# THUDM/GCC

Hardware: AMD Instinct MI355X
Metric: sampled-subgraphs/sec (higher is better)
Workload: dtype f32

## Files before the change

gcc_amd/_cabi.py:

```python
from __future__ import annotations

import ctypes
import os

_HERE = os.path.dirname(os.path.abspath(__file__))
LIB_PATH = os.path.join(_HERE, "csrc", "libgcc_amd.so")
HEADER_PATH = os.path.join(os.path.dirname(_HERE), "include", "gcc_amd.h")

c_i32p = ctypes.POINTER(ctypes.c_int32)
c_f32p = ctypes.POINTER(ctypes.c_float)
c_f64p = ctypes.POINTER(ctypes.c_double)

STATUS_SCRATCH_OVERFLOW = 1
STATUS_NODE_OVERFLOW = 2
STATUS_EDGE_OVERFLOW = 4


class GccGraph(ctypes.Structure):
    _fields_ = [
        ("row_ptr", ctypes.c_void_p),
        ("col_idx", ctypes.c_void_p),
        ("seed_cdf", ctypes.c_void_p),
        ("ltab", ctypes.c_void_p),
        ("num_nodes", ctypes.c_int64),
# ... 227 lines not shown
                                          ctypes.c_void_p, ctypes.c_void_p, ctypes.c_void_p, ctypes.c_void_p]),
    "gcc_posemb": (ctypes.c_int32, [ctypes.POINTER(GccBatchOut), ctypes.c_int32, ctypes.c_int32, ctypes.c_void_p,
                                    ctypes.c_void_p, ctypes.c_void_p, ctypes.c_uint64, ctypes.c_void_p, ctypes.c_int64, ctypes.c_void_p,
                                    ctypes.c_void_p, ctypes.c_void_p]),
    "gcc_gin_forward": (ctypes.c_int32, [ctypes.POINTER(GccGinPass), ctypes.c_int32, ctypes.c_void_p,
                                         ctypes.c_void_p]),
    "gcc_gin_forward_fetch": (ctypes.c_int32, [ctypes.POINTER(GccGinPass), ctypes.c_int32, ctypes.c_void_p, ctypes.c_void_p,
                                               ctypes.c_int32, ctypes.c_void_p, ctypes.c_void_p, ctypes.c_void_p]),
    "gcc_gin_backward_workspace_bytes": (ctypes.c_int64, [ctypes.c_int64, ctypes.c_int32, ctypes.c_int32]),
    "gcc_gin_backward": (ctypes.c_int32, [ctypes.POINTER(GccGinPass), ctypes.c_void_p, ctypes.POINTER(GccGinGrads),
                                          ctypes.c_int32, ctypes.c_void_p, ctypes.c_int64, ctypes.c_int64,
                                          ctypes.c_void_p, ctypes.c_void_p]),
    "gcc_gin_backward_sumsq": (ctypes.c_int32, [ctypes.POINTER(GccGinPass), ctypes.c_void_p, ctypes.POINTER(GccGinGrads),
                                                ctypes.c_void_p, ctypes.c_int64, ctypes.c_int64, ctypes.c_void_p, ctypes.c_int32,
                                                c_i32p, ctypes.c_void_p, ctypes.c_void_p]),
    "gcc_ginx_workspace_bytes": (ctypes.c_int64, [ctypes.c_int64, ctypes.c_int32, ctypes.c_int32, ctypes.c_int32, ctypes.c_int32, ctypes.c_int32]),
    "gcc_ginx_forward": (ctypes.c_int32, [ctypes.POINTER(GccGinxPass), ctypes.c_void_p]),
    "gcc_ginx_backward": (ctypes.c_int32, [ctypes.POINTER(GccGinxPass), ctypes.c_void_p, ctypes.POINTER(GccGinGrads), ctypes.c_void_p]),
    "gcc_ncex_forward": (ctypes.c_int32, [ctypes.c_void_p, ctypes.c_void_p, ctypes.c_void_p, ctypes.c_int32, ctypes.c_int32, ctypes.c_int32,
                                          ctypes.c_float, ctypes.c_int32] + [ctypes.c_void_p] * 8),
    "gcc_queue_enqueue_x": (ctypes.c_int32, [ctypes.c_void_p, ctypes.c_int32, ctypes.c_int32, ctypes.c_void_p, ctypes.c_int32, ctypes.c_int32,
                                             ctypes.c_void_p]),
    "gcc_ginw_forward": (ctypes.c_int32, [ctypes.POINTER(GccGinwArgs), ctypes.c_void_p, ctypes.c_void_p, ctypes.c_void_p]),
    "gcc_ginw_pack_weights": (ctypes.c_int32, [ctypes.c_void_p, ctypes.c_void_p, ctypes.c_int32, ctypes.c_void_p]),
    "gcc_nce_workspace_bytes": (ctypes.c_int64, [ctypes.c_int32, ctypes.c_int32]),
    "gcc_nce_forward": (ctypes.c_int32, [ctypes.POINTER(GccNceArgs), ctypes.c_void_p, ctypes.c_int64,
                                         ctypes.c_void_p, ctypes.c_void_p]),
    "gcc_nce_backward": (ctypes.c_int32, [ctypes.POINTER(GccNceArgs), ctypes.c_void_p, ctypes.c_int32,
                                          ctypes.c_void_p, ctypes.c_void_p, ctypes.c_int64, ctypes.c_void_p,
                                          ctypes.c_void_p]),
# ... 100 lines not shown
```

gcc_amd/csrc/encoder_bwd.hip:

```cpp
#include "encoder_common.h"

namespace {

constexpr int kWgChunks = 64;

struct BnCol { float mean, rstd, gamma, beta; };
__device__ __forceinline__ BnCol bn_col(const BnDev &bn, int c, double s1, double s2, double n, float eps)
{
    const double mean = s1 / n;
    double var = s2 / n - mean * mean;
    if (var < 0.0) var = 0.0;
    BnCol r;
    r.mean = (float)mean;
    r.rstd = (float)(1.0 / sqrt(var + (double)eps));
    r.gamma = bn.weight[c];
    r.beta = bn.bias[c];
    return r;
}

enum { RS = 0, RM = 1, PS = 2, PH = 3, K1 = 4, K2 = 5, K3 = 6, kCoefRows = 7 };

__device__ __forceinline__ void fill_coefs(float *C , const BnDev &bn, const double *bst, double n,
                                           float eps, double *scratch)
{
// ... 172 lines not shown
            g[cb] = gg;
            if (valid) st4(a.G + ((int64_t)i * a.B + b) * H + ch, gg);
        }
        f32x4 acc[4];
        mfma_rows16(g, wf, acc);
        if (valid) {
#pragma unroll
            for (int cb = 0; cb < 4; ++cb) {
                F4 o = {acc[cb][0], acc[cb][1], acc[cb][2], acc[cb][3]};
                st4(a.dpooled + ((int64_t)i * a.B + b) * H + 16 * cb + 4 * q, o);
            }
        }
    }
}

struct BwdCArgs {
    const int32_t *node_off, *row_ptr, *col_idx, *graph_id;
    const float *D;
    const float *dpooled;
    const float *z2;
    BnDev bnb, bnc;
    float *U;
    double *bst_c;
    int32_t B;
    float eps;
    int32_t cap;
};

#ifndef BWD_C_PER_CU
#define BWD_C_PER_CU 3
#endif
#ifndef BWD_GATHER_J
#define BWD_GATHER_J 8
#endif
__global__ __launch_bounds__(kThreads, BWD_C_PER_CU) void gin_bwd_c_kernel(BwdCArgs a)
{
    TRAIN_STEP_WAVE_PRIORITY();
    __shared__ float T[kTile * kLdt];
    __shared__ __attribute__((aligned(16))) float part[16 * 2 * H];
    __shared__ float Cb[kCoefRows * H], Cc[kCoefRows * H];
    __shared__ int prow[32];
    __shared__ int rpl[kTile + 1];
    const int tid = (int)threadIdx.x, t = tid & 15, gi = tid >> 4;
    int N;
    const float *Dp = a.D ? a.D : a.z2;
    auto ident = [&](int u) -> F4 { return ld4(Dp + (int64_t)u * H + 4 * t); };
    const int tf = first_tile();
    int gid4[kTile / 16], rp_own = 0;
    F4 own[kTile / 16], z4[kTile / 16];
    auto request = [&](int tile0) {
#pragma unroll
        for (int i = 0; i < kTile / 16; ++i) gid4[i] = a.graph_id[cap_row(tile0 + gi + 16 * i, a.cap)];
        rp_own = a.row_ptr[min(tile0 + min(tid, kTile), a.cap)];
#pragma unroll
        for (int i = 0; i < kTile / 16; ++i) own[i] = ident(cap_row(tile0 + gi + 16 * i, a.cap));
#pragma unroll
        for (int i = 0; i < kTile / 16; ++i) z4[i] = ld4(a.z2 + (int64_t)cap_row(tile0 + gi + 16 * i, a.cap) * H + 4 * t);
    };
    if (a.bnb.totals && a.bnc.totals) {
        const CoefReq rb = coef_request(a.bnb), rc = coef_request(a.bnc);
        const RepReq none = {};
        request(tf * kTile);
        N = a.node_off[a.B];
        SCHED_FENCE();
        if (no_tiles(N)) return;
        fill_coefs_from<false>(Cb, rb, none, (double)N, a.eps, (double *)part);
        fill_coefs_from<false>(Cc, rc, none, (double)N, a.eps, (double *)part);
        __syncthreads();
    } else {
        request(tf * kTile);
        N = ((const volatile int32_t *)a.node_off)[a.B];
        fill_coefs(Cb, a.bnb, nullptr, (double)N, a.eps, (double *)part);
        fill_coefs(Cc, a.bnc, nullptr, (double)N, a.eps, (double *)part);
    }
    F4 s1 = zero4(), s2 = zero4();
    bool any = false;
    for (TileWalk tw(N); tw.ti < tw.tend; tw.ti += tw.step) {
        const int tile0 = tw.ti * kTile;
        any = true;
        const int nrows = min(kTile, N - tile0);
        if (tw.ti != tf) request(tile0);
        F4 g4[kTile / 16];
        auto pooled_path = [&] {
#pragma unroll
            for (int i = 0; i < kTile / 16; ++i) g4[i] = ld4(a.dpooled + (int64_t)min(max(gid4[i], 0), a.B - 1) * H + 4 * t);
        };
        if (a.D) {
            if (tid <= nrows) rpl[tid] = rp_own;
#pragma unroll
            for (int i = 0; i < kTile / 16; ++i) st4(&T[(gi + 16 * i) * kLdt + 4 * t], gi + 16 * i < nrows ? own[i] : zero4());
            __syncthreads();
            gather_tile<BWD_GATHER_J>(T, part, prow, nrows, a.col_idx, ident, [](F4 x) { return x; }, 1.0f, rpl, pooled_path);
        } else {
            pooled_path();
        }
        {
            const F4 pbs = ld4(&Cb[PS * H + 4 * t]), pbh = ld4(&Cb[PH * H + 4 * t]);
            const F4 rcs = ld4(&Cc[RS * H + 4 * t]), rcm = ld4(&Cc[RM * H + 4 * t]);
            const F4 pcs = ld4(&Cc[PS * H + 4 * t]), pch = ld4(&Cc[PH * H + 4 * t]);
#pragma unroll
            for (int i = 0; i < kTile / 16; ++i) {
                const int r = gi + 16 * i, v = tile0 + r;
                if (r < nrows) {
                    F4 g = g4[i];
                    if (a.D) g = add4(g, ld4(&T[r * kLdt + 4 * t]));
                    const F4 y2 = relu4(fma4(z4[i], pbs, pbh));
                    const F4 yh = fma4(y2, rcs, rcm);
                    const F4 u = mask4(g, fma4(y2, pcs, pch));
                    st4(a.U + (int64_t)v * H + 4 * t, u);
                    s1 = add4(s1, u);
                    s2 = fma4(u, yh, s2);
                }
            }
        }
        __syncthreads();
    }
    if (!any) return;
    reduce_groups(part, s1, s2, a.bst_c, a.bst_c + H);
}

struct BwdBArgs {
    const int32_t *node_off;
    const float *U, *z2;
    BnDev bnb, bnc;
// ... 178 lines not shown
            else if (kMask) atomicAdd(&a.bst_out[rep + tid], v);
        }
        __syncthreads();
    }
}

constexpr int kEmbBlocks = 448;
constexpr int kEmbMaxElems = 10240;

struct EmbArgs {
    const int32_t *node_off, *row_ptr, *col_idx, *graph_id;
    const float *D, *dpooled0;
    float *demb_parts;
    int32_t B, pos_dim, emb_dim, max_degree;
    int32_t cap;
};

__global__ __launch_bounds__(kThreads) void gin_bwd_emb_kernel(EmbArgs a)
{
    TRAIN_STEP_WAVE_PRIORITY();
    __shared__ float T[kTile * kLdt];
    __shared__ float part[32 * H];
    __shared__ float E[kEmbMaxElems];
    __shared__ int dclrow[kTile], gidl[kTile];
    __shared__ int prow[32];
    __shared__ int rpl[kTile + 1];
    const int tid = (int)threadIdx.x, t = tid & 15, gi = tid >> 4;
    const bool my_cols = 4 * t + 3 >= a.pos_dim && 4 * t < a.pos_dim + a.emb_dim;
    auto ident = [&](int u) -> F4 { return my_cols ? ld4(a.D + (int64_t)u * H + 4 * t) : zero4(); };
    const int tf = first_tile();
    int rp_own, gid_own;
    F4 own[kTile / 16];
    auto request = [&](int tile0) {
        rp_own = a.row_ptr[min(tile0 + min(tid, kTile), a.cap)];
        gid_own = a.graph_id[cap_row(tile0 + (tid & (kTile - 1)), a.cap)];
#pragma unroll
        for (int i = 0; i < kTile / 16; ++i) own[i] = ident(cap_row(tile0 + gi + 16 * i, a.cap));
    };
    request(tf * kTile);
    const int N = a.node_off[a.B];
    SCHED_FENCE();
    const int elems = (a.max_degree + 1) * a.emb_dim;
    for (int i = tid; i < elems; i += kThreads) E[i] = 0.f;
    for (TileWalk tw(N); tw.ti < tw.tend; tw.ti += tw.step) {
        const int tile0 = tw.ti * kTile;
        const int nrows = min(kTile, N - tile0);
        {
            if (tw.ti != tf) request(tile0);
            if (tid <= nrows) rpl[tid] = rp_own;
            if (tid >= 128 && tid - 128 < nrows) gidl[tid - 128] = gid_own;
#pragma unroll
            for (int i = 0; i < kTile / 16; ++i) st4(&T[(gi + 16 * i) * kLdt + 4 * t], gi + 16 * i < nrows ? own[i] : zero4());
        }
        __syncthreads();
        constexpr int kIt = 4;
        const int total = nrows * a.emb_dim;
        int rr[kIt], cc[kIt];
        float dv[kIt];
        auto pooled_request = [&](int base) {
// ... 9 lines not shown
        if (tid < nrows) {
            const int deg = rpl[tid + 1] - rpl[tid];
            dclrow[tid] = deg < a.max_degree ? deg : a.max_degree;
        }
        for (int base = 0; base < total; base += kIt * kThreads) {
            if (base) pooled_request(base);
#pragma unroll
            for (int i = 0; i < kIt; ++i)
                if (base + tid + i * kThreads < total) T[rr[i] * kLdt + a.pos_dim + cc[i]] += dv[i];
        }
        __syncthreads();
        if (tid < a.emb_dim)
            for (int r = 0; r < nrows; ++r) E[dclrow[r] * a.emb_dim + tid] += T[r * kLdt + a.pos_dim + tid];
        __syncthreads();
    }
    for (int i = tid; i < elems; i += kThreads) a.demb_parts[(int64_t)blockIdx.x * elems + i] = E[i];
}

struct WgradJob {
    const float *dZ, *X;
    const double *Xd;
    BnDev bn;
    int32_t rows_fixed;
};
constexpr int kMaxWgJobs = 3 * GCC_GIN_MAX_LAYERS + 1;
struct WgradArgs {
    const int32_t *node_off;
    WgradJob job[kMaxWgJobs];
    float *slabs;
    float *bias_slabs;
    int32_t B;
    float eps;
    int32_t cap;
};

__global__ __launch_bounds__(kThreads, 3) void gin_wgrad_kernel(WgradArgs a)
{
    TRAIN_STEP_WAVE_PRIORITY();
    __shared__ float S[H * H];
    __shared__ float Cx[2 * H];
    const int jid = (int)blockIdx.y;
    const WgradJob &jb = a.job[jid];
    const int tid = (int)threadIdx.x, lane = lane_id(), wv = tid >> 6, j = lane & 15, q = lane >> 4;
    __shared__ float Sb[4 * H];
    const bool act = jb.bn.weight != nullptr;
    const bool fast = act && jb.bn.totals != nullptr;
    const int cc = tid & (H - 1);
    const double *tp = fast ? jb.bn.totals : (const double *)a.slabs;
    const float *wp = fast ? jb.bn.weight : a.slabs, *bp = fast ? jb.bn.bias : a.slabs;
    const CoefReq cr = {tp[cc], tp[H + cc], wp[cc], bp[cc]};
    const int rcap = jb.rows_fixed > 0 ? jb.rows_fixed : a.cap;
    f32x4 acc[4][4];
    float bsum[4] = {0.f, 0.f, 0.f, 0.f};
#pragma unroll
    for (int ob = 0; ob < 4; ++ob)
#pragma unroll
        for (int kb = 0; kb < 4; ++kb) { f32x4 z = {0.f, 0.f, 0.f, 0.f}; acc[ob][kb] = z; }
    float av[4][4], xv[4][4];
    const bool xdouble = jb.Xd != nullptr;
    auto fetch = [&](int tile0, float (&A)[4][4], float (&X)[4][4]) {
        int64_t off[4];
#pragma unroll
        for (int s = 0; s < 4; ++s) {
            const int row = tile0 + 16 * wv + 4 * s + q;
            off[s] = (int64_t)cap_row(row, rcap) * H + j;
#pragma unroll
            for (int k = 0; k < 4; ++k) A[s][k] = jb.dZ[off[s] + 16 * k];
        }
        if (xdouble) {
#pragma unroll
            for (int h = 0; h < 4; h += 2) {
                double xd[2][4];
#pragma unroll
                for (int s = 0; s < 2; ++s)
#pragma unroll
                    for (int k = 0; k < 4; ++k) xd[s][k] = jb.Xd[off[h + s] + 16 * k];
#pragma unroll
                for (int s = 0; s < 2; ++s)
#pragma unroll
                    for (int k = 0; k < 4; ++k) X[h + s][k] = (float)xd[s][k];
            }
        } else {
#pragma unroll
            for (int s = 0; s < 4; ++s)
#pragma unroll
                for (int k = 0; k < 4; ++k) X[s][k] = jb.X[off[s] + 16 * k];
        }
    };
    auto mask_tile = [&](int tile0, int N, float (&A)[4][4], float (&X)[4][4]) {
#pragma unroll
        for (int s = 0; s < 4; ++s) {
            const bool in = tile0 + 16 * wv + 4 * s + q < N;
#pragma unroll
            for (int k = 0; k < 4; ++k) { A[s][k] = in ? A[s][k] : 0.f; X[s][k] = in ? X[s][k] : 0.f; }
        }
    };
    const int tf = first_tile();
    fetch(tf * kTile, av, xv);
    const int Nn = a.node_off[a.B];
    SCHED_FENCE();
    const int N = jb.rows_fixed > 0 ? jb.rows_fixed : Nn;
    TileWalk tw(N);
    if (tid < H) {
        float sc = 1.f, sh = 0.f;
        if (fast) {
            const double mean = cr.s1 / (double)Nn;
            double var = cr.s2 / (double)Nn - mean * mean;
            if (var < 0.0) var = 0.0;
            const double rstd = 1.0 / sqrt(var + (double)a.eps);
            sc = (float)((double)cr.gamma * rstd);
            sh = (float)((double)cr.beta - mean * (double)cr.gamma * rstd);
        } else if (act) {
            bn_scale_shift(jb.bn, tid, (double)Nn, a.eps, 1, sc, sh);
        }
        Cx[tid] = sc;
        Cx[H + tid] = sh;
    }
    __syncthreads();
    float xs[4], xh[4];
#pragma unroll
    for (int kb = 0; kb < 4; ++kb) { xs[kb] = Cx[16 * kb + j]; xh[kb] = Cx[H + 16 * kb + j]; }
    for (; tw.ti < tw.tend; tw.ti += tw.step) {
        const int tile0 = tw.ti * kTile;
        float an[4][4], xn[4][4];
        const bool more = tw.ti + tw.step < tw.tend;
        if (more) fetch((tw.ti + tw.step) * kTile, an, xn);
        mask_tile(tile0, N, av, xv);
#pragma unroll
        for (int s = 0; s < 4; ++s) {
            const int row = tile0 + 16 * wv + 4 * s + q;
            float bv[4];
#pragma unroll
            for (int k = 0; k < 4; ++k) {
                bsum[k] += av[s][k];
                bv[k] = act ? (row < N ? fmaxf(fmaf(xv[s][k], xs[k], xh[k]), 0.f) : 0.f) : xv[s][k];
            }
#pragma unroll
            for (int ob = 0; ob < 4; ++ob)
#pragma unroll
                for (int kb = 0; kb < 4; ++kb) acc[ob][kb] = mfma_16x16x4_f32(av[s][ob], bv[kb], acc[ob][kb]);
        }
        if (more) {
#pragma unroll
            for (int s = 0; s < 4; ++s)
#pragma unroll
                for (int k = 0; k < 4; ++k) { av[s][k] = an[s][k]; xv[s][k] = xn[s][k]; }
        }
    }
    for (int w = 0; w < 4; ++w) {
        if (wv == w) {
#pragma unroll
            for (int ob = 0; ob < 4; ++ob)
#pragma unroll
                for (int kb = 0; kb < 4; ++kb)
#pragma unroll
                    for (int r = 0; r < 4; ++r) {
                        const int o = 16 * ob + 4 * q + r, k = 16 * kb + j;
                        S[o * H + k] = (w == 0 ? 0.f : S[o * H + k]) + acc[ob][kb][r];
                    }
        }
        __syncthreads();
    }
    float *slab = a.slabs + ((int64_t)jid * kWgChunks + blockIdx.x) * H * H;
    for (int i = tid; i < H * H; i += kThreads) slab[i] = S[i];
#pragma unroll
    for (int k = 0; k < 4; ++k) {
        bsum[k] += wave_shfl_xor(bsum[k], 16);
        bsum[k] += wave_shfl_xor(bsum[k], 32);
        if (q == 0) Sb[wv * H + 16 * k + j] = bsum[k];
    }
    __syncthreads();
    if (tid < H)
        a.bias_slabs[((int64_t)jid * kWgChunks + blockIdx.x) * H + tid] =
            (Sb[tid] + Sb[H + tid]) + (Sb[2 * H + tid] + Sb[3 * H + tid]);
}

struct FinalArgs {
    const float *slabs, *bias_slabs;
    const double *bst;
    const float *demb_parts;
    gcc_gin_grads g;
    int32_t B, L, kdim0, emb_rows, emb_dim, accumulate, hid;
    double *sumsq_parts;
};

__device__ __forceinline__ float put(float *dst, float v, int acc)
{
    if (!dst) return 0.f;
    const float w = acc ? *dst + v : v;
// ... 114 lines not shown
    w.total = o;
    return w;
}

}

extern "C" int64_t gcc_gin_backward_workspace_bytes(int64_t node_cap, int32_t batch_size, int32_t num_gin_layers)
{
    if (node_cap <= 0 || batch_size <= 0 || num_gin_layers < 1 || num_gin_layers > GCC_GIN_MAX_LAYERS) {
        snprintf(g_err, kErrLen, "gcc_gin_backward_workspace_bytes: bad argument");
        return -1;
    }
    return bwd_layout(nullptr, node_cap, batch_size, num_gin_layers, kEmbMaxElems).total;
}

static int32_t gin_backward_launches(const gcc_gin_pass *pass, const float *dfeat, const gcc_gin_grads *grads,
                                     int32_t accumulate, void *workspace, int64_t workspace_bytes,
                                     int64_t node_cap, double *sumsq_parts, int32_t parts_cap, int32_t *nparts,
                                     gcc_prof *prof, void *stream)
{
    if (!pass || !dfeat || !grads || !workspace) {
        snprintf(g_err, kErrLen, "gcc_gin_backward: null argument");
        return -1;
    }
    const gcc_gin_pass &p = *pass;
    if (p.edge_multiplicity > 1) {
        snprintf(g_err, kErrLen, "gcc_gin_backward: edge_multiplicity %d (inference-only feature)", p.edge_multiplicity);
        return -2;
    }
    const int L = p.w.num_gin_layers, B = p.batch_size;
// ... 8 lines not shown
    const BwdWork w = bwd_layout((char *)workspace, node_cap, B, L, kEmbMaxElems);
    if (workspace_bytes < w.total) {
        snprintf(g_err, kErrLen, "gcc_gin_backward: workspace %lld < %lld bytes", (long long)workspace_bytes,
                 (long long)w.total);
        return -3;
    }
    if (node_cap < 1 || node_cap > 0x7fffffff || (p.node_cap > 0 && p.node_cap != node_cap)) {
        snprintf(g_err, kErrLen, "gcc_gin_backward: node_cap %lld (the pass says %lld)", (long long)node_cap, (long long)p.node_cap);
        return -2;
    }
    const int32_t cap = (int32_t)node_cap;
    hipStream_t s = (hipStream_t)stream;
    prof_mark(prof, 0, s);
    const dim3 grid(tile_grid(p.rows_hint > 0 && p.rows_hint < node_cap ? p.rows_hint : node_cap)), block(kThreads);
    auto bst = [&](int l, int which) { return w.bst + ((int64_t)l * 3 + which) * kRep * 3 * H; };
    {
        ReadBwdArgs a;
        a.dfeat = dfeat; a.score = p.score; a.feat = p.feat; a.drop = drop_cfg(p);
        for (int i = 0; i <= L; ++i) a.pred_w[i] = p.w.pred_w[i];
        a.G = w.G; a.dpooled = w.dpooled; a.B = B; a.nlayers = L; a.kdim0 = kdim0; a.normalize = p.normalize; a.hid = hidden_of(p.w);
        a.norm_eps = p.w.norm_eps;
        a.zero = (float4 *)((char *)workspace + w.off_zero); a.zero16 = w.zero_bytes / 16; a.nread = ((B + 15) / 16 * (L + 1) + 3) / 4;
        hipLaunchKernelGGL(gin_bwd_readout_kernel, dim3(a.nread + 64), block, 0, s, a);
    }
    for (int l = L - 1; l >= 0; --l) {
        const BnDev bna = bn_of(p, p.w.bn_a[l], l, 0);
        const BnDev bnb = bn_of(p, p.w.bn_b[l], l, 1);
        const BnDev bnc = bn_of(p, p.w.bn_c[l], l, 2);
        {
            BwdCArgs a = {p.node_off, p.row_ptr, p.col_idx, p.graph_id, l == L - 1 ? nullptr : w.D,
                          w.dpooled + (int64_t)(l + 1) * B * H, p.z2[l], bnb, bnc, w.U, bst(l, 2), B, p.w.bn_eps, cap};
            hipLaunchKernelGGL(gin_bwd_c_kernel, grid, block, 0, s, a);
        }
        {
            BwdBArgs a = {p.node_off, w.U, p.z2[l], bnb, bnc, bst(l, 2), w.V, bst(l, 1), B, p.w.bn_eps, cap};
            hipLaunchKernelGGL(gin_bwd_b_kernel, grid, block, 0, s, a);
        }
        {
            BwdLinArgs a = {p.node_off, w.V, p.z2[l], bnb, bst(l, 1), bst(l, 1) + 2 * H, p.w.lin1_w[l], hidden_of(p.w),
                            w.dz2[l], w.Wt, p.z1[l], bna, bst(l, 0), B, p.w.bn_eps, cap};
            hipLaunchKernelGGL((gin_bwd_lin_kernel<true>), grid, block, 0, s, a);
        }
        {
            BwdLinArgs a = {p.node_off, w.Wt, p.z1[l], bna, bst(l, 0), bst(l, 0) + 2 * H, p.w.lin0_w[l],
                            l == 0 ? kdim0 : hidden_of(p.w), w.dz1[l], w.D, nullptr, BnDev(), nullptr, B, p.w.bn_eps, cap};
            hipLaunchKernelGGL((gin_bwd_lin_kernel<false>), grid, block, 0, s, a);
        }
    }
    {
        EmbArgs a = {p.node_off, p.row_ptr, p.col_idx, p.graph_id, w.D, w.dpooled, w.demb_parts, B, p.w.pos_dim,
                     p.w.deg_emb_dim, p.w.max_degree, cap};
        hipLaunchKernelGGL(gin_bwd_emb_kernel, dim3(kEmbBlocks), block, 0, s, a);
    }
    {
        WgradArgs a;
        a.node_off = p.node_off; a.slabs = w.slabs; a.bias_slabs = w.bias_slabs; a.B = B; a.eps = p.w.bn_eps; a.cap = cap;
        for (int l = 0; l < L; ++l) {
            a.job[2 * l + 0] = {w.dz1[l], p.agg[l], nullptr, BnDev(), 0};
            a.job[2 * l + 1] = {w.dz2[l], p.z1[l], nullptr, bn_of(p, p.w.bn_a[l], l, 0), 0};
        }
        for (int i = 0; i <= L; ++i)
            a.job[2 * L + i] = {w.G + (int64_t)i * B * H, nullptr, p.pooled + (int64_t)i * B * H, BnDev(), B};
        hipLaunchKernelGGL(gin_wgrad_kernel, dim3(kWgChunks, 3 * L + 1), block, 0, s, a);
    }
    {
        FinalArgs a;
        a.slabs = w.slabs; a.bias_slabs = w.bias_slabs; a.bst = w.bst; a.demb_parts = w.demb_parts; a.g = *grads;
        a.B = B; a.L = L; a.kdim0 = kdim0; a.emb_rows = p.w.max_degree + 1; a.emb_dim = p.w.deg_emb_dim; a.hid = hidden_of(p.w);
        a.accumulate = accumulate;
        const int64_t upto4 = (int64_t)(3 * L + 1) * H * H + (int64_t)(L + 1) * H + (int64_t)L * 9 * H;
        const int64_t total = ((upto4 + 63) & ~(int64_t)63) + (((int64_t)a.emb_rows * a.emb_dim * 8 + 63) & ~(int64_t)63);
        const int64_t blocks = (total + kThreads - 1) / kThreads;
        a.sumsq_parts = sumsq_parts;
        if (sumsq_parts) {
            if (blocks > parts_cap) {
                snprintf(g_err, kErrLen, "gcc_gin_backward_sumsq: %lld partials, room for %d", (long long)blocks, parts_cap);
                return -3;
// ... 34 lines not shown
```

gcc_amd/csrc/encoder_common.h:

```cpp
#pragma once
#include "host_common.h"

namespace {

constexpr int H = GCC_GIN_HIDDEN;
constexpr int kTile = 64;
constexpr int kLdt = 72;
constexpr int kThreads = 256;
constexpr int kGridX = 768;
constexpr int kMaxPass = 2;
#ifndef GCC_KREP
#define GCC_KREP GCC_GIN_STAT_REPLICAS
#endif
constexpr int kRep = GCC_KREP;

__device__ __forceinline__ int first_tile()
{
    const int b = (int)blockIdx.x;
    if (((int)gridDim.x & 31) != 0) return b;
    const int x = b & 7, j = b >> 3;
    return ((((j >> 2) << 3) + x) << 2) + (j & 3);
}
struct TileWalk {
    int ti, tend, step;
    __device__ __forceinline__ explicit TileWalk(int N) : ti(first_tile()), tend((N + kTile - 1) / kTile), step((int)gridDim.x) {}
};
__device__ __forceinline__ bool no_tiles(int N) { return first_tile() * kTile >= N; }
__device__ __forceinline__ int cap_row(int row, int cap) { return min(row, cap - 1); }

struct F4 { float x, y, z, w; };

__device__ __forceinline__ F4 ld4(const float *p)
{
    const float4 v = *reinterpret_cast<const float4 *>(p);
    F4 r = {v.x, v.y, v.z, v.w};
    return r;
}
__device__ __forceinline__ void st4(float *p, F4 v)
{
    *reinterpret_cast<float4 *>(p) = make_float4(v.x, v.y, v.z, v.w);
}
__device__ __forceinline__ F4 add4(F4 a, F4 b) { F4 r = {a.x + b.x, a.y + b.y, a.z + b.z, a.w + b.w}; return r; }
// ... 366 lines not shown
{
    const int tid = (int)threadIdx.x;
    if (tid < 2 * H) {
        const double v = (double)red[tid] + (double)red[128 + tid] + (double)red[256 + tid] + (double)red[384 + tid];
        atomicAdd(&stats[((int)blockIdx.x % kRep) * 2 * H + tid], v);
    }
}


#ifndef GATHER_DBG
#define GATHER_DBG 0
#endif
template <int kGatherJ, class Load, class Xform, class Overlap>
__device__ __forceinline__ void gather_tile(float *T, float *part , int *prow , int nrows,
                                            const int32_t *col_idx, Load load, Xform xform, float nbr_weight,
                                            const int *rp_lds , Overlap overlap)
{
    const int tid = (int)threadIdx.x, t = tid & 15, gi = tid >> 4, gbase = lane_id() & ~15;
    const int ebeg = rp_lds[0], eend = rp_lds[nrows];
    const int chunk = (eend - ebeg + 15) >> 4;
    const int e0 = ebeg + gi * chunk, e1 = min(e0 + chunk, eend);
    if (t < 2) prow[gi * 2 + t] = -1;
    F4 acc = {0.f, 0.f, 0.f, 0.f};
    int cur = -1, first = -1;
    auto flush = [&](bool last) {
        if (cur < 0) return;
        if (cur == first || last) {
            const int slot = gi * 2 + (cur == first ? 0 : 1);
            st4(&part[slot * H + 4 * t], acc);
            if (t == 0) prow[slot] = cur;
        } else {
            float *dst = &T[cur * kLdt + 4 * t];
            const F4 self = ld4(dst);
// ... 149 lines not shown
```

include/gcc_amd.h:

```cpp
#ifndef GCC_AMD_H
#define GCC_AMD_H

#include <stdint.h>

#ifdef __cplusplus
extern "C" {
#endif

#define GCC_AMD_ABI_VERSION 3

#define GCC_STATUS_SCRATCH_OVERFLOW 1
#define GCC_STATUS_NODE_OVERFLOW    2
#define GCC_STATUS_EDGE_OVERFLOW    4

int32_t gcc_abi_version(void);
const char *gcc_last_error(void);

typedef struct gcc_prof gcc_prof;
gcc_prof *gcc_prof_create(int32_t num_marks);
void gcc_prof_destroy(gcc_prof *p);
int32_t gcc_prof_elapsed_ms(gcc_prof *p, int32_t from_mark, int32_t to_mark, float *ms);

int32_t gcc_stream_create_cu_mask(const uint32_t *cu_mask, int32_t words, void **stream);
int32_t gcc_debug_load(int32_t kind, int32_t workgroups, int32_t threads, int32_t lds_bytes, int64_t ticks, int32_t max_iters,
// ... 169 lines not shown
    float *bn_b_w[GCC_GIN_MAX_LAYERS], *bn_b_b[GCC_GIN_MAX_LAYERS];
    float *bn_c_w[GCC_GIN_MAX_LAYERS], *bn_c_b[GCC_GIN_MAX_LAYERS];
    float *pred_w[GCC_GIN_MAX_LAYERS + 1], *pred_b[GCC_GIN_MAX_LAYERS + 1];
} gcc_gin_grads;

int64_t gcc_gin_backward_workspace_bytes(int64_t node_cap, int32_t batch_size, int32_t num_gin_layers);

int32_t gcc_gin_backward(const gcc_gin_pass *pass, const float *dfeat, const gcc_gin_grads *grads,
                         int32_t accumulate, void *workspace, int64_t workspace_bytes, int64_t node_cap,
                         gcc_prof *prof, void *stream);

int32_t gcc_gin_backward_sumsq(const gcc_gin_pass *pass, const float *dfeat, const gcc_gin_grads *grads, void *workspace,
                               int64_t workspace_bytes, int64_t node_cap, double *sumsq_parts, int32_t parts_cap,
                               int32_t *nparts, gcc_prof *prof, void *stream);

typedef struct gcc_ginx_pass {
    const int32_t *node_off, *row_ptr, *col_idx, *graph_id;
    const float *pos;
    const int32_t *seed_local;
    int32_t batch_size;
    int32_t training;
    int32_t update_running_stats;
    int32_t normalize;
    const float *dropout_keep;
    int32_t hidden, out_dim;
    int32_t edge_multiplicity;
    int32_t reserved_;
    int64_t node_cap;
    gcc_gin_weights w;
    void *workspace;
// ... 177 lines not shown
```

Before: 717,400.

## Fold weight-gradient work into backward chain kernels as extra rider workgroups

Moves the separate weight-gradient GEMM kernel into the GIN backward chain. Extra 'rider' workgroups are appended to the bwd_c and bwd_emb launches and compute the wgrad slabs for jobs whose inputs are already available. This removes one kernel launch and lets the small reduction GEMMs overlap with the latency-bound gather kernels. It also adds inline-asm scalar-register hints and extends the tile-walk helpers so chain blocks index by offset. The risks are more LDS and register pressure in the chain kernels and possible contention with the critical-path work.

```diff
diff --git a/gcc_amd/_cabi.py b/gcc_amd/_cabi.py
--- a/gcc_amd/_cabi.py
+++ b/gcc_amd/_cabi.py
@@ -265,6 +265,7 @@
     "gcc_gin_backward_sumsq": (ctypes.c_int32, [ctypes.POINTER(GccGinPass), ctypes.c_void_p, ctypes.POINTER(GccGinGrads),
                                                 ctypes.c_void_p, ctypes.c_int64, ctypes.c_int64, ctypes.c_void_p, ctypes.c_int32,
                                                 c_i32p, ctypes.c_void_p, ctypes.c_void_p]),
+    "gcc_gin_bwd_riders_set": (ctypes.c_int32, [ctypes.c_int32]),
     "gcc_ginx_workspace_bytes": (ctypes.c_int64, [ctypes.c_int64, ctypes.c_int32, ctypes.c_int32, ctypes.c_int32, ctypes.c_int32, ctypes.c_int32]),
     "gcc_ginx_forward": (ctypes.c_int32, [ctypes.POINTER(GccGinxPass), ctypes.c_void_p]),
     "gcc_ginx_backward": (ctypes.c_int32, [ctypes.POINTER(GccGinxPass), ctypes.c_void_p, ctypes.POINTER(GccGinGrads), ctypes.c_void_p]),
diff --git a/gcc_amd/csrc/encoder_bwd.hip b/gcc_amd/csrc/encoder_bwd.hip
--- a/gcc_amd/csrc/encoder_bwd.hip
+++ b/gcc_amd/csrc/encoder_bwd.hip
@@ -210,6 +210,191 @@
     }
 }
 
+struct WgradJob {
+    const float *dZ, *X;
+    const double *Xd;
+    BnDev bn;
+    int32_t rows_fixed;
+};
+constexpr int kMaxWgJobs = 3 * GCC_GIN_MAX_LAYERS + 1;
+struct WgradArgs {
+    const int32_t *node_off;
+    WgradJob job[kMaxWgJobs];
+    float *slabs;
+    float *bias_slabs;
+    int32_t B;
+    float eps;
+    int32_t cap;
+};
+constexpr int kMaxRideJobs = kMaxWgJobs - 2;
+static_assert(kWgChunks % kRep == 0 && kWgChunks % 8 == 0, "riders in front of the chain keep its workgroups' statistics replica and XCD");
+struct WgradRide {
+    WgradJob job[kMaxRideJobs];
+    float *slabs, *bias_slabs;
+    int32_t jid0;
+    float eps;
+    int32_t first;
+};
+
+struct WgradCtx {
+    const int32_t *node_off;
+    float *slabs, *bias_slabs;
+    int32_t B;
+    float eps;
+    int32_t cap;
+};
+__device__ __forceinline__ void wgrad_chunk(const WgradCtx &a, const WgradJob &jb, int jid, int chunk, float *S, float *Cx, float *Sb)
+{
+    const int tid = (int)threadIdx.x, lane = lane_id(), wv = tid >> 6, j = lane & 15, q = lane >> 4;
+    const bool act = jb.bn.weight != nullptr;
+    const bool fast = act && jb.bn.totals != nullptr;
+    const int cc = tid & (H - 1);
+    const double *tp = fast ? jb.bn.totals : (const double *)a.slabs;
+    const float *wp = fast ? jb.bn.weight : a.slabs, *bp = fast ? jb.bn.bias : a.slabs;
+    const CoefReq cr = {tp[cc], tp[H + cc], wp[cc], bp[cc]};
+    const int rcap = jb.rows_fixed > 0 ? jb.rows_fixed : a.cap;
+    f32x4 acc[4][4];
+    float bsum[4] = {0.f, 0.f, 0.f, 0.f};
+#pragma unroll
+    for (int ob = 0; ob < 4; ++ob)
+#pragma unroll
+        for (int kb = 0; kb < 4; ++kb) { f32x4 z = {0.f, 0.f, 0.f, 0.f}; acc[ob][kb] = z; }
+    float av[4][4], xv[4][4];
+    const bool xdouble = jb.Xd != nullptr;
+    auto fetch = [&](int tile0, float (&A)[4][4], float (&X)[4][4]) {
+        int64_t off[4];
+#pragma unroll
+        for (int s = 0; s < 4; ++s) {
+            const int row = tile0 + 16 * wv + 4 * s + q;
+            off[s] = (int64_t)cap_row(row, rcap) * H + j;
+#pragma unroll
+            for (int k = 0; k < 4; ++k) A[s][k] = jb.dZ[off[s] + 16 * k];
+        }
+        if (xdouble) {
+#pragma unroll
+            for (int h = 0; h < 4; h += 2) {
+                double xd[2][4];
+#pragma unroll
+                for (int s = 0; s < 2; ++s)
+#pragma unroll
+                    for (int k = 0; k < 4; ++k) xd[s][k] = jb.Xd[off[h + s] + 16 * k];
+#pragma unroll
+                for (int s = 0; s < 2; ++s)
+#pragma unroll
+                    for (int k = 0; k < 4; ++k) X[h + s][k] = (float)xd[s][k];
+            }
+        } else {
+#pragma unroll
+            for (int s = 0; s < 4; ++s)
+#pragma unroll
+                for (int k = 0; k < 4; ++k) X[s][k] = jb.X[off[s] + 16 * k];
+        }
+    };
+    auto mask_tile = [&](int tile0, int N, float (&A)[4][4], float (&X)[4][4]) {
+#pragma unroll
+        for (int s = 0; s < 4; ++s) {
+            const bool in = tile0 + 16 * wv + 4 * s + q < N;
+#pragma unroll
+            for (int k = 0; k < 4; ++k) { A[s][k] = in ? A[s][k] : 0.f; X[s][k] = in ? X[s][k] : 0.f; }
+        }
+    };
+    const int tf = first_tile_of(chunk, kWgChunks);
+    fetch(tf * kTile, av, xv);
+    const int Nn = a.node_off[a.B];
+    SCHED_FENCE();
+    const int N = jb.rows_fixed > 0 ? jb.rows_fixed : Nn;
+    TileWalk tw(N, chunk, kWgChunks);
+    if (tid < H) {
+        float sc = 1.f, sh = 0.f;
+        if (fast) {
+            const double mean = cr.s1 / (double)Nn;
+            double var = cr.s2 / (double)Nn - mean * mean;
+            if (var < 0.0) var = 0.0;
+            const double rstd = 1.0 / sqrt(var + (double)a.eps);
+            sc = (float)((double)cr.gamma * rstd);
+            sh = (float)((double)cr.beta - mean * (double)cr.gamma * rstd);
+        } else if (act) {
+            bn_scale_shift(jb.bn, tid, (double)Nn, a.eps, 1, sc, sh);
+        }
+        Cx[tid] = sc;
+        Cx[H + tid] = sh;
+    }
+    __syncthreads();
+    float xs[4], xh[4];
+#pragma unroll
+    for (int kb = 0; kb < 4; ++kb) { xs[kb] = Cx[16 * kb + j]; xh[kb] = Cx[H + 16 * kb + j]; }
+    for (; tw.ti < tw.tend; tw.ti += tw.step) {
+        const int tile0 = tw.ti * kTile;
+        float an[4][4], xn[4][4];
+        const bool more = tw.ti + tw.step < tw.tend;
+        if (more) fetch((tw.ti + tw.step) * kTile, an, xn);
+        mask_tile(tile0, N, av, xv);
+#pragma unroll
+        for (int s = 0; s < 4; ++s) {
+            const int row = tile0 + 16 * wv + 4 * s + q;
+            float bv[4];
+#pragma unroll
+            for (int k = 0; k < 4; ++k) {
+                bsum[k] += av[s][k];
+                bv[k] = act ? (row < N ? fmaxf(fmaf(xv[s][k], xs[k], xh[k]), 0.f) : 0.f) : xv[s][k];
+            }
+#pragma unroll
+            for (int ob = 0; ob < 4; ++ob)
+#pragma unroll
+                for (int kb = 0; kb < 4; ++kb) acc[ob][kb] = mfma_16x16x4_f32(av[s][ob], bv[kb], acc[ob][kb]);
+        }
+        if (more) {
+#pragma unroll
+            for (int s = 0; s < 4; ++s)
+#pragma unroll
+                for (int k = 0; k < 4; ++k) { av[s][k] = an[s][k]; xv[s][k] = xn[s][k]; }
+        }
+    }
+    for (int w = 0; w < 4; ++w) {
+        if (wv == w) {
+#pragma unroll
+            for (int ob = 0; ob < 4; ++ob)
+#pragma unroll
+                for (int kb = 0; kb < 4; ++kb)
+#pragma unroll
+                    for (int r = 0; r < 4; ++r) {
+                        const int o = 16 * ob + 4 * q + r, k = 16 * kb + j;
+                        S[o * H + k] = (w == 0 ? 0.f : S[o * H + k]) + acc[ob][kb][r];
+                    }
+        }
+        __syncthreads();
+    }
+    float *slab = a.slabs + ((int64_t)jid * kWgChunks + chunk) * H * H;
+    for (int i = tid; i < H * H; i += kThreads) slab[i] = S[i];
+#pragma unroll
+    for (int k = 0; k < 4; ++k) {
+        bsum[k] += wave_shfl_xor(bsum[k], 16);
+        bsum[k] += wave_shfl_xor(bsum[k], 32);
+        if (q == 0) Sb[wv * H + 16 * k + j] = bsum[k];
+    }
+    __syncthreads();
+    if (tid < H)
+        a.bias_slabs[((int64_t)jid * kWgChunks + chunk) * H + tid] =
+            (Sb[tid] + Sb[H + tid]) + (Sb[2 * H + tid] + Sb[3 * H + tid]);
+}
+
+__global__ __launch_bounds__(kThreads, 3) void gin_wgrad_kernel(WgradArgs a)
+{
+    TRAIN_STEP_WAVE_PRIORITY();
+    __shared__ float S[H * H];
+    __shared__ float Cx[2 * H];
+    __shared__ float Sb[4 * H];
+    const WgradCtx c = {a.node_off, a.slabs, a.bias_slabs, a.B, a.eps, a.cap};
+    wgrad_chunk(c, a.job[blockIdx.y], (int)blockIdx.y, (int)blockIdx.x, S, Cx, Sb);
+}
+
+__device__ __forceinline__ void wgrad_ride(const WgradRide &rd, const int32_t *node_off, int B, int cap, int r, float *S, float *small)
+{
+    const int jl = wave_uniform(r / kWgChunks);
+    const WgradCtx c = {node_off, rd.slabs, rd.bias_slabs, B, rd.eps, cap};
+    wgrad_chunk(c, rd.job[jl], rd.jid0 + jl, r % kWgChunks, S, small, small + 2 * H);
+}
+
 struct BwdCArgs {
     const int32_t *node_off, *row_ptr, *col_idx, *graph_id;
     const float *D;
@@ -221,6 +406,8 @@
     int32_t B;
     float eps;
     int32_t cap;
+    int32_t chain;
+    WgradRide ride;
 };
 
 #ifndef BWD_C_PER_CU
@@ -237,21 +424,36 @@
     __shared__ float Cb[kCoefRows * H], Cc[kCoefRows * H];
     __shared__ int prow[32];
     __shared__ int rpl[kTile + 1];
-    const int tid = (int)threadIdx.x, t = tid & 15, gi = tid >> 4;
+    const int32_t *row_ptr = a.row_ptr, *col_idx = a.col_idx, *graph_id = a.graph_id;
+    const float *D = a.D, *dpooled = a.dpooled, *z2 = a.z2;
+    float *U = a.U;
+    float eps = a.eps;
+    int cap = a.cap;
+    SCALAR_ARGS_HERE(SLIST(SKEEP(row_ptr), SKEEP(col_idx), SKEEP(graph_id), SKEEP(D), SKEEP(dpooled), SKEEP(z2), SKEEP(U), SKEEP(eps),
+                           SKEEP(cap)),
+                     SARG(a.node_off), SARG(a.bnb.weight), SARG(a.bnb.bias), SARG(a.bnb.totals), SARG(a.bnc.weight),
+                     SARG(a.bnc.bias), SARG(a.bnc.totals), SARG(a.bst_c), SARG(a.B), SARG(a.chain), SARG(a.ride.first));
+    const int nchain = a.chain, wg = (int)blockIdx.x - a.ride.first;
+    if (wg < 0 || wg >= nchain) {
+        static_assert(sizeof(T) >= H * H * sizeof(float) && sizeof(part) >= 6 * H * sizeof(float), "the rider's S / Cx / Sb");
+        wgrad_ride(a.ride, a.node_off, a.B, a.cap, wg < 0 ? (int)blockIdx.x : (int)blockIdx.x - nchain, T, part);
+        return;
+    }
+    int tid = (int)threadIdx.x, t = tid & 15, gi = tid >> 4;
     int N;
-    const float *Dp = a.D ? a.D : a.z2;
+    const float *Dp = D ? D : z2;
     auto ident = [&](int u) -> F4 { return ld4(Dp + (int64_t)u * H + 4 * t); };
-    const int tf = first_tile();
+    const int tf = first_tile_of(wg, nchain);
     int gid4[kTile / 16], rp_own = 0;
     F4 own[kTile / 16], z4[kTile / 16];
     auto request = [&](int tile0) {
 #pragma unroll
-        for (int i = 0; i < kTile / 16; ++i) gid4[i] = a.graph_id[cap_row(tile0 + gi + 16 * i, a.cap)];
-        rp_own = a.row_ptr[min(tile0 + min(tid, kTile), a.cap)];
-#pragma unroll
-        for (int i = 0; i < kTile / 16; ++i) own[i] = ident(cap_row(tile0 + gi + 16 * i, a.cap));
-#pragma unroll
-        for (int i = 0; i < kTile / 16; ++i) z4[i] = ld4(a.z2 + (int64_t)cap_row(tile0 + gi + 16 * i, a.cap) * H + 4 * t);
+        for (int i = 0; i < kTile / 16; ++i) gid4[i] = graph_id[cap_row(tile0 + gi + 16 * i, cap)];
+        rp_own = row_ptr[min(tile0 + min(tid, kTile), cap)];
+#pragma unroll
+        for (int i = 0; i < kTile / 16; ++i) own[i] = ident(cap_row(tile0 + gi + 16 * i, cap));
+#pragma unroll
+        for (int i = 0; i < kTile / 16; ++i) z4[i] = ld4(z2 + (int64_t)cap_row(tile0 + gi + 16 * i, cap) * H + 4 * t);
     };
     if (a.bnb.totals && a.bnc.totals) {
         const CoefReq rb = coef_request(a.bnb), rc = coef_request(a.bnc);
@@ -259,34 +461,39 @@
         request(tf * kTile);
         N = a.node_off[a.B];
         SCHED_FENCE();
-        if (no_tiles(N)) return;
-        fill_coefs_from<false>(Cb, rb, none, (double)N, a.eps, (double *)part);
-        fill_coefs_from<false>(Cc, rc, none, (double)N, a.eps, (double *)part);
+        if (no_tiles_of(N, wg, nchain)) return;
+        fill_coefs_from<false>(Cb, rb, none, (double)N, eps, (double *)part);
+        fill_coefs_from<false>(Cc, rc, none, (double)N, eps, (double *)part);
         __syncthreads();
     } else {
         request(tf * kTile);
         N = ((const volatile int32_t *)a.node_off)[a.B];
-        fill_coefs(Cb, a.bnb, nullptr, (double)N, a.eps, (double *)part);
-        fill_coefs(Cc, a.bnc, nullptr, (double)N, a.eps, (double *)part);
+        fill_coefs(Cb, a.bnb, nullptr, (double)N, eps, (double *)part);
+        fill_coefs(Cc, a.bnc, nullptr, (double)N, eps, (double *)part);
     }
     F4 s1 = zero4(), s2 = zero4();
     bool any = false;
-    for (TileWalk tw(N); tw.ti < tw.tend; tw.ti += tw.step) {
+    for (TileWalk tw(N, wg, nchain); tw.ti < tw.tend; tw.ti += tw.step) {
         const int tile0 = tw.ti * kTile;
         any = true;
+        {
+            uint32_t tid_ = threadIdx.x;
+            opaque_u32(tid_);
+            tid = (int)tid_; t = tid & 15; gi = tid >> 4;
+        }
         const int nrows = min(kTile, N - tile0);
         if (tw.ti != tf) request(tile0);
         F4 g4[kTile / 16];
         auto pooled_path = [&] {
 #pragma unroll
-            for (int i = 0; i < kTile / 16; ++i) g4[i] = ld4(a.dpooled + (int64_t)min(max(gid4[i], 0), a.B - 1) * H + 4 * t);
+            for (int i = 0; i < kTile / 16; ++i) g4[i] = ld4(dpooled + (int64_t)min(max(gid4[i], 0), a.B - 1) * H + 4 * t);
         };
-        if (a.D) {
+        if (D) {
             if (tid <= nrows) rpl[tid] = rp_own;
 #pragma unroll
             for (int i = 0; i < kTile / 16; ++i) st4(&T[(gi + 16 * i) * kLdt + 4 * t], gi + 16 * i < nrows ? own[i] : zero4());
             __syncthreads();
-            gather_tile<BWD_GATHER_J>(T, part, prow, nrows, a.col_idx, ident, [](F4 x) { return x; }, 1.0f, rpl, pooled_path);
+            gather_tile<BWD_GATHER_J>(T, part, prow, nrows, col_idx, ident, [](F4 x) { return x; }, 1.0f, rpl, pooled_path, tid, tid & 63);
         } else {
             pooled_path();
         }
@@ -299,11 +506,11 @@
                 const int r = gi + 16 * i, v = tile0 + r;
                 if (r < nrows) {
                     F4 g = g4[i];
-                    if (a.D) g = add4(g, ld4(&T[r * kLdt + 4 * t]));
+                    if (D) g = add4(g, ld4(&T[r * kLdt + 4 * t]));
                     const F4 y2 = relu4(fma4(z4[i], pbs, pbh));
                     const F4 yh = fma4(y2, rcs, rcm);
                     const F4 u = mask4(g, fma4(y2, pcs, pch));
-                    st4(a.U + (int64_t)v * H + 4 * t, u);
+                    st4(U + (int64_t)v * H + 4 * t, u);
                     s1 = add4(s1, u);
                     s2 = fma4(u, yh, s2);
                 }
@@ -512,6 +719,8 @@
     float *demb_parts;
     int32_t B, pos_dim, emb_dim, max_degree;
     int32_t cap;
+    int32_t chain;
+    WgradRide ride;
 };
 
 __global__ __launch_bounds__(kThreads) void gin_bwd_emb_kernel(EmbArgs a)
@@ -523,10 +732,19 @@
     __shared__ int dclrow[kTile], gidl[kTile];
     __shared__ int prow[32];
     __shared__ int rpl[kTile + 1];
+    SCALAR_ARGS_HERE(, SARG(a.node_off), SARG(a.row_ptr), SARG(a.col_idx), SARG(a.graph_id), SARG(a.D), SARG(a.dpooled0),
+                     SARG(a.demb_parts), SARG(a.B), SARG(a.pos_dim), SARG(a.emb_dim), SARG(a.max_degree), SARG(a.cap), SARG(a.chain),
+                     SARG(a.ride.first));
+    const int nchain = a.chain, wg = (int)blockIdx.x - a.ride.first;
+    if (wg < 0 || wg >= nchain) {
+        static_assert(sizeof(T) >= H * H * sizeof(float) && sizeof(part) >= 6 * H * sizeof(float), "the rider's S / Cx / Sb");
+        wgrad_ride(a.ride, a.node_off, a.B, a.cap, wg < 0 ? (int)blockIdx.x : (int)blockIdx.x - nchain, T, part);
+        return;
+    }
     const int tid = (int)threadIdx.x, t = tid & 15, gi = tid >> 4;
     const bool my_cols = 4 * t + 3 >= a.pos_dim && 4 * t < a.pos_dim + a.emb_dim;
     auto ident = [&](int u) -> F4 { return my_cols ? ld4(a.D + (int64_t)u * H + 4 * t) : zero4(); };
-    const int tf = first_tile();
+    const int tf = first_tile_of(wg, nchain);
     int rp_own, gid_own;
     F4 own[kTile / 16];
     auto request = [&](int tile0) {
@@ -540,7 +758,7 @@
     SCHED_FENCE();
     const int elems = (a.max_degree + 1) * a.emb_dim;
     for (int i = tid; i < elems; i += kThreads) E[i] = 0.f;
-    for (TileWalk tw(N); tw.ti < tw.tend; tw.ti += tw.step) {
+    for (TileWalk tw(N, wg, nchain); tw.ti < tw.tend; tw.ti += tw.step) {
         const int tile0 = tw.ti * kTile;
         const int nrows = min(kTile, N - tile0);
         {
@@ -580,165 +798,7 @@
             for (int r = 0; r < nrows; ++r) E[dclrow[r] * a.emb_dim + tid] += T[r * kLdt + a.pos_dim + tid];
         __syncthreads();
     }
-    for (int i = tid; i < elems; i += kThreads) a.demb_parts[(int64_t)blockIdx.x * elems + i] = E[i];
-}
-
-struct WgradJob {
-    const float *dZ, *X;
-    const double *Xd;
-    BnDev bn;
-    int32_t rows_fixed;
-};
-constexpr int kMaxWgJobs = 3 * GCC_GIN_MAX_LAYERS + 1;
-struct WgradArgs {
-    const int32_t *node_off;
-    WgradJob job[kMaxWgJobs];
-    float *slabs;
-    float *bias_slabs;
-    int32_t B;
-    float eps;
-    int32_t cap;
-};
-
-__global__ __launch_bounds__(kThreads, 3) void gin_wgrad_kernel(WgradArgs a)
-{
-    TRAIN_STEP_WAVE_PRIORITY();
-    __shared__ float S[H * H];
-    __shared__ float Cx[2 * H];
-    const int jid = (int)blockIdx.y;
-    const WgradJob &jb = a.job[jid];
-    const int tid = (int)threadIdx.x, lane = lane_id(), wv = tid >> 6, j = lane & 15, q = lane >> 4;
-    __shared__ float Sb[4 * H];
-    const bool act = jb.bn.weight != nullptr;
-    const bool fast = act && jb.bn.totals != nullptr;
-    const int cc = tid & (H - 1);
-    const double *tp = fast ? jb.bn.totals : (const double *)a.slabs;
-    const float *wp = fast ? jb.bn.weight : a.slabs, *bp = fast ? jb.bn.bias : a.slabs;
-    const CoefReq cr = {tp[cc], tp[H + cc], wp[cc], bp[cc]};
-    const int rcap = jb.rows_fixed > 0 ? jb.rows_fixed : a.cap;
-    f32x4 acc[4][4];
-    float bsum[4] = {0.f, 0.f, 0.f, 0.f};
-#pragma unroll
-    for (int ob = 0; ob < 4; ++ob)
-#pragma unroll
-        for (int kb = 0; kb < 4; ++kb) { f32x4 z = {0.f, 0.f, 0.f, 0.f}; acc[ob][kb] = z; }
-    float av[4][4], xv[4][4];
-    const bool xdouble = jb.Xd != nullptr;
-    auto fetch = [&](int tile0, float (&A)[4][4], float (&X)[4][4]) {
-        int64_t off[4];
-#pragma unroll
-        for (int s = 0; s < 4; ++s) {
-            const int row = tile0 + 16 * wv + 4 * s + q;
-            off[s] = (int64_t)cap_row(row, rcap) * H + j;
-#pragma unroll
-            for (int k = 0; k < 4; ++k) A[s][k] = jb.dZ[off[s] + 16 * k];
-        }
-        if (xdouble) {
-#pragma unroll
-            for (int h = 0; h < 4; h += 2) {
-                double xd[2][4];
-#pragma unroll
-                for (int s = 0; s < 2; ++s)
-#pragma unroll
-                    for (int k = 0; k < 4; ++k) xd[s][k] = jb.Xd[off[h + s] + 16 * k];
-#pragma unroll
-                for (int s = 0; s < 2; ++s)
-#pragma unroll
-                    for (int k = 0; k < 4; ++k) X[h + s][k] = (float)xd[s][k];
-            }
-        } else {
-#pragma unroll
-            for (int s = 0; s < 4; ++s)
-#pragma unroll
-                for (int k = 0; k < 4; ++k) X[s][k] = jb.X[off[s] + 16 * k];
-        }
-    };
-    auto mask_tile = [&](int tile0, int N, float (&A)[4][4], float (&X)[4][4]) {
-#pragma unroll
-        for (int s = 0; s < 4; ++s) {
-            const bool in = tile0 + 16 * wv + 4 * s + q < N;
-#pragma unroll
-            for (int k = 0; k < 4; ++k) { A[s][k] = in ? A[s][k] : 0.f; X[s][k] = in ? X[s][k] : 0.f; }
-        }
-    };
-    const int tf = first_tile();
-    fetch(tf * kTile, av, xv);
-    const int Nn = a.node_off[a.B];
-    SCHED_FENCE();
-    const int N = jb.rows_fixed > 0 ? jb.rows_fixed : Nn;
-    TileWalk tw(N);
-    if (tid < H) {
-        float sc = 1.f, sh = 0.f;
-        if (fast) {
-            const double mean = cr.s1 / (double)Nn;
-            double var = cr.s2 / (double)Nn - mean * mean;
-            if (var < 0.0) var = 0.0;
-            const double rstd = 1.0 / sqrt(var + (double)a.eps);
-            sc = (float)((double)cr.gamma * rstd);
-            sh = (float)((double)cr.beta - mean * (double)cr.gamma * rstd);
-        } else if (act) {
-            bn_scale_shift(jb.bn, tid, (double)Nn, a.eps, 1, sc, sh);
-        }
-        Cx[tid] = sc;
-        Cx[H + tid] = sh;
-    }
-    __syncthreads();
-    float xs[4], xh[4];
-#pragma unroll
-    for (int kb = 0; kb < 4; ++kb) { xs[kb] = Cx[16 * kb + j]; xh[kb] = Cx[H + 16 * kb + j]; }
-    for (; tw.ti < tw.tend; tw.ti += tw.step) {
-        const int tile0 = tw.ti * kTile;
-        float an[4][4], xn[4][4];
-        const bool more = tw.ti + tw.step < tw.tend;
-        if (more) fetch((tw.ti + tw.step) * kTile, an, xn);
-        mask_tile(tile0, N, av, xv);
-#pragma unroll
-        for (int s = 0; s < 4; ++s) {
-            const int row = tile0 + 16 * wv + 4 * s + q;
-            float bv[4];
-#pragma unroll
-            for (int k = 0; k < 4; ++k) {
-                bsum[k] += av[s][k];
-                bv[k] = act ? (row < N ? fmaxf(fmaf(xv[s][k], xs[k], xh[k]), 0.f) : 0.f) : xv[s][k];
-            }
-#pragma unroll
-            for (int ob = 0; ob < 4; ++ob)
-#pragma unroll
-                for (int kb = 0; kb < 4; ++kb) acc[ob][kb] = mfma_16x16x4_f32(av[s][ob], bv[kb], acc[ob][kb]);
-        }
-        if (more) {
-#pragma unroll
-            for (int s = 0; s < 4; ++s)
-#pragma unroll
-                for (int k = 0; k < 4; ++k) { av[s][k] = an[s][k]; xv[s][k] = xn[s][k]; }
-        }
-    }
-    for (int w = 0; w < 4; ++w) {
-        if (wv == w) {
-#pragma unroll
-            for (int ob = 0; ob < 4; ++ob)
-#pragma unroll
-                for (int kb = 0; kb < 4; ++kb)
-#pragma unroll
-                    for (int r = 0; r < 4; ++r) {
-                        const int o = 16 * ob + 4 * q + r, k = 16 * kb + j;
-                        S[o * H + k] = (w == 0 ? 0.f : S[o * H + k]) + acc[ob][kb][r];
-                    }
-        }
-        __syncthreads();
-    }
-    float *slab = a.slabs + ((int64_t)jid * kWgChunks + blockIdx.x) * H * H;
-    for (int i = tid; i < H * H; i += kThreads) slab[i] = S[i];
-#pragma unroll
-    for (int k = 0; k < 4; ++k) {
-        bsum[k] += wave_shfl_xor(bsum[k], 16);
-        bsum[k] += wave_shfl_xor(bsum[k], 32);
-        if (q == 0) Sb[wv * H + 16 * k + j] = bsum[k];
-    }
-    __syncthreads();
-    if (tid < H)
-        a.bias_slabs[((int64_t)jid * kWgChunks + blockIdx.x) * H + tid] =
-            (Sb[tid] + Sb[H + tid]) + (Sb[2 * H + tid] + Sb[3 * H + tid]);
+    for (int i = tid; i < elems; i += kThreads) a.demb_parts[(int64_t)wg * elems + i] = E[i];
 }
 
 struct FinalArgs {
@@ -883,6 +943,20 @@
     return bwd_layout(nullptr, node_cap, batch_size, num_gin_layers, kEmbMaxElems).total;
 }
 
+constexpr int kBwdRidersDefault = 1;
+static int g_bwd_riders = -1;
+static int bwd_riders_mode()
+{
+    if (g_bwd_riders < 0) { const char *e = getenv("GCC_BWD_RIDERS"); g_bwd_riders = e ? atoi(e) : kBwdRidersDefault; }
+    return g_bwd_riders < 0 || g_bwd_riders > 3 ? kBwdRidersDefault : g_bwd_riders;
+}
+extern "C" int32_t gcc_gin_bwd_riders_set(int32_t on)
+{
+    const int32_t was = bwd_riders_mode();
+    g_bwd_riders = on < 0 ? -1 : on;
+    return was;
+}
+
 static int32_t gin_backward_launches(const gcc_gin_pass *pass, const float *dfeat, const gcc_gin_grads *grads,
                                      int32_t accumulate, void *workspace, int64_t workspace_bytes,
                                      int64_t node_cap, double *sumsq_parts, int32_t parts_cap, int32_t *nparts,
@@ -921,6 +995,23 @@
     prof_mark(prof, 0, s);
     const dim3 grid(tile_grid(p.rows_hint > 0 && p.rows_hint < node_cap ? p.rows_hint : node_cap)), block(kThreads);
     auto bst = [&](int l, int which) { return w.bst + ((int64_t)l * 3 + which) * kRep * 3 * H; };
+    WgradJob job[kMaxWgJobs];
+    for (int l = 0; l < L; ++l) {
+        job[2 * l + 0] = {w.dz1[l], p.agg[l], nullptr, BnDev(), 0};
+        job[2 * l + 1] = {w.dz2[l], p.z1[l], nullptr, bn_of(p, p.w.bn_a[l], l, 0), 0};
+    }
+    for (int i = 0; i <= L; ++i)
+        job[2 * L + i] = {w.G + (int64_t)i * B * H, nullptr, p.pooled + (int64_t)i * B * H, BnDev(), B};
+    const int mode = bwd_riders_mode();
+    const bool riders = mode != 0;
+    auto ride = [&](WgradRide &r, int jid0, int njobs, int front_jobs) -> unsigned {
+        r = WgradRide();
+        if (!riders || njobs <= 0) return 0;
+        for (int i = 0; i < njobs; ++i) r.job[i] = job[jid0 + i];
+        r.slabs = w.slabs; r.bias_slabs = w.bias_slabs; r.jid0 = jid0; r.eps = p.w.bn_eps;
+        r.first = front_jobs * kWgChunks;
+        return (unsigned)(njobs * kWgChunks);
+    };
     {
         ReadBwdArgs a;
         a.dfeat = dfeat; a.score = p.score; a.feat = p.feat; a.drop = drop_cfg(p);
@@ -936,8 +1027,12 @@
         const BnDev bnc = bn_of(p, p.w.bn_c[l], l, 2);
         {
             BwdCArgs a = {p.node_off, p.row_ptr, p.col_idx, p.graph_id, l == L - 1 ? nullptr : w.D,
-                          w.dpooled + (int64_t)(l + 1) * B * H, p.z2[l], bnb, bnc, w.U, bst(l, 2), B, p.w.bn_eps, cap};
-            hipLaunchKernelGGL(gin_bwd_c_kernel, grid, block, 0, s, a);
+                          w.dpooled + (int64_t)(l + 1) * B * H, p.z2[l], bnb, bnc, w.U, bst(l, 2), B, p.w.bn_eps, cap, (int32_t)grid.x};
+            unsigned nride;
+            if (mode == 3) nride = l == 0 ? ride(a.ride, 2, 3 * L - 1, 2 * L - 2) : 0;
+            else if (l == L - 1) nride = ride(a.ride, 2 * L, L + 1, mode == 2 ? L + 1 : 0);
+            else nride = ride(a.ride, 2 * (l + 1), 2, mode == 2 ? 2 : 0);
+            hipLaunchKernelGGL(gin_bwd_c_kernel, dim3(grid.x + nride), block, 0, s, a);
         }
         {
             BwdBArgs a = {p.node_off, w.U, p.z2[l], bnb, bnc, bst(l, 2), w.V, bst(l, 1), B, p.w.bn_eps, cap};
@@ -956,18 +1051,14 @@
     }
     {
         EmbArgs a = {p.node_off, p.row_ptr, p.col_idx, p.graph_id, w.D, w.dpooled, w.demb_parts, B, p.w.pos_dim,
-                     p.w.deg_emb_dim, p.w.max_degree, cap};
-        hipLaunchKernelGGL(gin_bwd_emb_kernel, dim3(kEmbBlocks), block, 0, s, a);
-    }
-    {
+                     p.w.deg_emb_dim, p.w.max_degree, cap, kEmbBlocks};
+        const unsigned nride = ride(a.ride, 0, 2, mode == 1 ? 0 : 2);
+        hipLaunchKernelGGL(gin_bwd_emb_kernel, dim3(kEmbBlocks + nride), block, 0, s, a);
+    }
+    if (!riders) {
         WgradArgs a;
         a.node_off = p.node_off; a.slabs = w.slabs; a.bias_slabs = w.bias_slabs; a.B = B; a.eps = p.w.bn_eps; a.cap = cap;
-        for (int l = 0; l < L; ++l) {
-            a.job[2 * l + 0] = {w.dz1[l], p.agg[l], nullptr, BnDev(), 0};
-            a.job[2 * l + 1] = {w.dz2[l], p.z1[l], nullptr, bn_of(p, p.w.bn_a[l], l, 0), 0};
-        }
-        for (int i = 0; i <= L; ++i)
-            a.job[2 * L + i] = {w.G + (int64_t)i * B * H, nullptr, p.pooled + (int64_t)i * B * H, BnDev(), B};
+        for (int i = 0; i < 3 * L + 1; ++i) a.job[i] = job[i];
         hipLaunchKernelGGL(gin_wgrad_kernel, dim3(kWgChunks, 3 * L + 1), block, 0, s, a);
     }
     {
diff --git a/gcc_amd/csrc/encoder_common.h b/gcc_amd/csrc/encoder_common.h
--- a/gcc_amd/csrc/encoder_common.h
+++ b/gcc_amd/csrc/encoder_common.h
@@ -14,18 +14,32 @@
 #endif
 constexpr int kRep = GCC_KREP;
 
-__device__ __forceinline__ int first_tile()
-{
-    const int b = (int)blockIdx.x;
-    if (((int)gridDim.x & 31) != 0) return b;
+#ifdef GCC_AMD_HIPEMU
+#define SCALAR_ARGS_HERE(KEPT, ...) ((void)0)
+#define SLIST(...) 0
+#define SARG(x) 0
+#define SKEEP(x) 0
+#else
+#define SCALAR_ARGS_HERE(KEPT, ...) asm volatile("" : KEPT : __VA_ARGS__)
+#define SLIST(...) __VA_ARGS__
+#define SARG(x) "s"(x)
+#define SKEEP(x) "+s"(x)
+#endif
+
+__device__ __forceinline__ int first_tile_of(int b, int n)
+{
+    if ((n & 31) != 0) return b;
     const int x = b & 7, j = b >> 3;
     return ((((j >> 2) << 3) + x) << 2) + (j & 3);
 }
+__device__ __forceinline__ int first_tile() { return first_tile_of((int)blockIdx.x, (int)gridDim.x); }
 struct TileWalk {
     int ti, tend, step;
     __device__ __forceinline__ explicit TileWalk(int N) : ti(first_tile()), tend((N + kTile - 1) / kTile), step((int)gridDim.x) {}
+    __device__ __forceinline__ TileWalk(int N, int b, int n) : ti(first_tile_of(b, n)), tend((N + kTile - 1) / kTile), step(n) {}
 };
 __device__ __forceinline__ bool no_tiles(int N) { return first_tile() * kTile >= N; }
+__device__ __forceinline__ bool no_tiles_of(int N, int b, int n) { return first_tile_of(b, n) * kTile >= N; }
 __device__ __forceinline__ int cap_row(int row, int cap) { return min(row, cap - 1); }
 
 struct F4 { float x, y, z, w; };
@@ -422,9 +436,10 @@
 template <int kGatherJ, class Load, class Xform, class Overlap>
 __device__ __forceinline__ void gather_tile(float *T, float *part , int *prow , int nrows,
                                             const int32_t *col_idx, Load load, Xform xform, float nbr_weight,
-                                            const int *rp_lds , Overlap overlap)
-{
-    const int tid = (int)threadIdx.x, t = tid & 15, gi = tid >> 4, gbase = lane_id() & ~15;
+                                            const int *rp_lds , Overlap overlap,
+                                            int tid = (int)threadIdx.x, int lane = lane_id())
+{
+    const int t = tid & 15, gi = tid >> 4, gbase = lane & ~15;
     const int ebeg = rp_lds[0], eend = rp_lds[nrows];
     const int chunk = (eend - ebeg + 15) >> 4;
     const int e0 = ebeg + gi * chunk, e1 = min(e0 + chunk, eend);
diff --git a/include/gcc_amd.h b/include/gcc_amd.h
--- a/include/gcc_amd.h
+++ b/include/gcc_amd.h
@@ -207,6 +207,8 @@
                                int64_t workspace_bytes, int64_t node_cap, double *sumsq_parts, int32_t parts_cap,
                                int32_t *nparts, gcc_prof *prof, void *stream);
 
+int32_t gcc_gin_bwd_riders_set(int32_t on);
+
 typedef struct gcc_ginx_pass {
     const int32_t *node_off, *row_ptr, *col_idx, *graph_id;
     const float *pos;
```

Result: no change. 713,400 (-0.6%).
